# changhaonan/A3VLM

Hardware: AMD Instinct MI355X
Metric: image-text samples/sec (train) + articulation-decode tok/s (higher is better)
Workload: dtype bf16

## Files before the change

a3vlm_amd/csrc/a3v_train.hip:

```cpp
#include "a3v_common.h"

namespace {

template <typename T>
__global__ __launch_bounds__(256) void transpose_kernel(const T* __restrict__ src, int64_t lds_, int64_t bs_s,
                                                        T* __restrict__ dst, int64_t ldd, int64_t bs_d, int R, int C, int Rpad) {
  __shared__ T tile[64][64 + 2];
  const T* s = src + blockIdx.z * bs_s;
  T* d = dst + blockIdx.z * bs_d;
  const int r0 = blockIdx.y * 64, c0 = blockIdx.x * 64;
  const int tx = threadIdx.x & 63, ty = threadIdx.x >> 6;
  for (int i = ty; i < 64; i += 4) {
    const int r = r0 + i, c = c0 + tx;
    tile[i][tx] = (r < R && c < C) ? s[(int64_t)r * lds_ + c] : (T)0.f;
  }
  __syncthreads();
  for (int i = ty; i < 64; i += 4) {
    const int c = c0 + i, r = r0 + tx;
    if (c < C && r < Rpad) d[(int64_t)c * ldd + r] = tile[tx][i];
  }
}

__global__ __launch_bounds__(256) void transpose_bf16_vec_kernel(const bf16_t* __restrict__ src, int64_t lds_, int64_t bs_s,
                                                                 bf16_t* __restrict__ dst, int64_t ldd, int64_t bs_d, int R, int C, int Rpad,
// ... 75 lines not shown
        Cvt<TS>::st(dhr + c, Cvt<TS>::ld(dhr + c) + (r * dyv * w[c] - xv * k2));
        dwp[i] += dyv * xv * r;
      }
    }
  }
  if (dw) {
#pragma unroll
    for (int i = 0; i < MAXC; ++i) {
      const int c = tid + i * 256;
      if (c < dim) atomicAdd(dw + c, dwp[i]);
    }
  }
}


template <typename TA, int RPB, int MAXV, bool PART, typename TS = float>
__global__ __launch_bounds__(256) void rmsnorm_bwd_vec_kernel(const TS* __restrict__ x, int64_t ldx, const float* __restrict__ w,
                                                              const TA* __restrict__ dy, int64_t lddy, TS* __restrict__ dh,
                                                              int64_t lddh, float* __restrict__ dw, int rows, int dim, float eps,
                                                              bf16_t* __restrict__ dh_bf = nullptr, int64_t ld_bf = 0) {
  __shared__ float red[2][8];
  const int tid = threadIdx.x;
  const int nv = dim >> 2;
  f32x4 wv[MAXV], dwp[MAXV];
#pragma unroll
  for (int i = 0; i < MAXV; ++i) {
    const int c = tid + i * 256;
    wv[i] = c < nv ? reinterpret_cast<const f32x4*>(w)[c] : f32x4{0.f, 0.f, 0.f, 0.f};
    dwp[i] = f32x4{0.f, 0.f, 0.f, 0.f};
  }
  const int row0 = blockIdx.x * RPB;
#ifdef RMSB_NO_PREFETCH
  constexpr bool PF = false;
#else
  constexpr bool PF = sizeof(TS) == 2 && sizeof(TA) == 2 && MAXV > 4;
#endif
  bf16x4 nx[MAXV], ng[MAXV], nh[MAXV];
  auto fetch = [&](int row) {
    if constexpr (PF) {
      const int rc = row < rows ? row : rows - 1;
#pragma unroll
      for (int i = 0; i < MAXV; ++i) {
        const int c = tid + i * 256;
        const int cc = c < nv ? c : 0;
        nx[i] = *reinterpret_cast<const bf16x4*>(reinterpret_cast<const bf16_t*>(x) + (int64_t)rc * ldx + 4 * cc);
        ng[i] = *reinterpret_cast<const bf16x4*>(reinterpret_cast<const bf16_t*>(dy) + (int64_t)rc * lddy + 4 * cc);
        nh[i] = *reinterpret_cast<const bf16x4*>(reinterpret_cast<const bf16_t*>(dh) + (int64_t)rc * lddh + 4 * cc);
      }
    }
  };
  fetch(row0);
  for (int rr = 0; rr < RPB; ++rr) {
    const int row = row0 + rr;
    if (row >= rows) break;
    const TS* xr = x + (int64_t)row * ldx;
    const TA* dyr = dy + (int64_t)row * lddy;
    f32x4 xv[MAXV], gv[MAXV], hv[MAXV];
    float s1 = 0.f, s2 = 0.f;
#pragma unroll
    for (int i = 0; i < MAXV; ++i) {
      const int c = tid + i * 256;
      if (c < nv) {
        if constexpr (PF) {
#pragma unroll
          for (int e = 0; e < 4; ++e) { xv[i][e] = (float)nx[i][e]; gv[i][e] = (float)ng[i][e]; hv[i][e] = (float)nh[i][e]; }
        } else {
        if constexpr (sizeof(TS) == 2) {
          const bf16x4 xb = *reinterpret_cast<const bf16x4*>(xr + 4 * c);
#pragma unroll
          for (int e = 0; e < 4; ++e) xv[i][e] = (float)xb[e];
        } else {
          xv[i] = *reinterpret_cast<const f32x4*>(xr + 4 * c);
        }
        if constexpr (sizeof(TA) == 2) {
          const bf16x4 d = *reinterpret_cast<const bf16x4*>(dyr + 4 * c);
#pragma unroll
          for (int e = 0; e < 4; ++e) gv[i][e] = (float)d[e];
        } else {
          gv[i] = *reinterpret_cast<const f32x4*>(dyr + 4 * c);
        }
        }
      } else {
        xv[i] = f32x4{0.f, 0.f, 0.f, 0.f};
        gv[i] = f32x4{0.f, 0.f, 0.f, 0.f};
      }
#pragma unroll
      for (int e = 0; e < 4; ++e) {
        s1 = fmaf(xv[i][e], xv[i][e], s1);
        s2 = fmaf(gv[i][e] * wv[i][e], xv[i][e], s2);
      }
    }
    if (rr + 1 < RPB) fetch(row + 1);
    s1 = wave_sum(s1); s2 = wave_sum(s2);
    const int pb = rr & 1;
    if ((tid & 63) == 0) { red[pb][tid >> 6] = s1; red[pb][4 + (tid >> 6)] = s2; }
    __syncthreads();
    s1 = red[pb][0] + red[pb][1] + red[pb][2] + red[pb][3];
    s2 = red[pb][4] + red[pb][5] + red[pb][6] + red[pb][7];
    const float r = rsqrtf(s1 / (float)dim + eps);
    const float k2 = r * r * r * s2 / (float)dim;
    TS* dhr = dh + (int64_t)row * lddh;
#pragma unroll
    for (int i = 0; i < MAXV; ++i) {
      const int c = tid + i * 256;
      if (c < nv) {
        f32x4 o;
        if constexpr (PF) {
          o = hv[i];
        } else if constexpr (sizeof(TS) == 2) {
          const bf16x4 ob0 = *reinterpret_cast<const bf16x4*>(dhr + 4 * c);
#pragma unroll
          for (int e = 0; e < 4; ++e) o[e] = (float)ob0[e];
        } else {
          o = *reinterpret_cast<const f32x4*>(dhr + 4 * c);
        }
#pragma unroll
        for (int e = 0; e < 4; ++e) {
          o[e] += r * gv[i][e] * wv[i][e] - xv[i][e] * k2;
          dwp[i][e] += gv[i][e] * xv[i][e] * r;
        }
        if constexpr (sizeof(TS) == 2) {
          bf16x4 ob1;
// ... 21 lines not shown
        if (c < nv) out[c] = dwp[i];
      }
    } else {
#pragma unroll
      for (int i = 0; i < MAXV; ++i) {
        const int c = tid + i * 256;
        if (c < nv) {
#pragma unroll
          for (int e = 0; e < 4; ++e) atomicAdd(dw + 4 * c + e, dwp[i][e]);
        }
      }
    }
  }
}

__global__ __launch_bounds__(256) void colsum_add_kernel(const float* __restrict__ part, int nrows, int cols, float* __restrict__ out) {
  const int c = blockIdx.x * 256 + threadIdx.x;
  if (c >= cols) return;
  const int per = (nrows + gridDim.y - 1) / gridDim.y;
  const int r0 = blockIdx.y * per, r1 = min(nrows, r0 + per);
  float a0 = 0.f, a1 = 0.f, a2 = 0.f, a3 = 0.f;
  int r = r0;
  for (; r + 4 <= r1; r += 4) {
    a0 += part[(int64_t)r * cols + c];
    a1 += part[(int64_t)(r + 1) * cols + c];
    a2 += part[(int64_t)(r + 2) * cols + c];
    a3 += part[(int64_t)(r + 3) * cols + c];
  }
  for (; r < r1; ++r) a0 += part[(int64_t)r * cols + c];
  if (r1 > r0) atomicAdd(out + c, (a0 + a1) + (a2 + a3));
}

template <typename TA, int RPB, typename TD = float>
__global__ __launch_bounds__(256) void layernorm_bwd_kernel(const TA* __restrict__ x, int64_t ldx, const float* __restrict__ w,
                                                            const TD* __restrict__ dy, int64_t lddy, const int32_t* __restrict__ row_map,
                                                            TA* __restrict__ dx, int64_t lddx, float* __restrict__ dw, float* __restrict__ db,
                                                            int rows, int dim, float eps) {
  __shared__ float red[12];
  const int tid = threadIdx.x;
  constexpr int MAXC = 32;
  float dwp[MAXC], dbp[MAXC];
#pragma unroll
  for (int i = 0; i < MAXC; ++i) { dwp[i] = 0.f; dbp[i] = 0.f; }
  const int row0 = blockIdx.x * RPB;
  for (int rr = 0; rr < RPB; ++rr) {
// ... 415 lines not shown
static int rmsnorm_bwd_impl(const TS* x, int64_t ldx, const float* w, const void* dy, int64_t lddy, TS* dh, int64_t lddh,
                            float* dw, float* dw_scratch, int rows, int dim, float eps, int act_dtype, void* stream, bf16_t* dh_bf,
                            int64_t ld_bf) {
  if (!x || !w || !dy || !dh || rows <= 0) return A3V_ERR_ARG;
  if (dim > 8192) return A3V_ERR_SHAPE;
  constexpr uintptr_t SMASK = sizeof(TS) == 2 ? 7 : 15;
  if (dim % 4 == 0 && ldx % 4 == 0 && lddy % 4 == 0 && lddh % 4 == 0 && (act_dtype == A3V_BF16 || act_dtype == A3V_F32) &&
      ((reinterpret_cast<uintptr_t>(x) | reinterpret_cast<uintptr_t>(dh)) & SMASK) == 0 && (reinterpret_cast<uintptr_t>(w) & 15) == 0 &&
      (reinterpret_cast<uintptr_t>(dy) & (act_dtype == A3V_BF16 ? 7 : 15)) == 0) {
    constexpr int RV = 8;
    const int nb = (rows + RV - 1) / RV;
    dim3 gv(nb);
    const bool part = dw && dw_scratch && (reinterpret_cast<uintptr_t>(dw_scratch) & 15) == 0;
    float* dwo = part ? dw_scratch : dw;
#define A3V_RB(TT, MV, PP) hipLaunchKernelGGL((rmsnorm_bwd_vec_kernel<TT, RV, MV, PP, TS>), gv, dim3(256), 0, ST, x, ldx, w, (const TT*)dy, lddy, dh, lddh, dwo, rows, dim, eps, dh_bf, ld_bf)
    if (dim <= 4096) {
      if (act_dtype == A3V_BF16) { if (part) A3V_RB(bf16_t, 4, true); else A3V_RB(bf16_t, 4, false); }
      else { if (part) A3V_RB(float, 4, true); else A3V_RB(float, 4, false); }
    } else {
      if (act_dtype == A3V_BF16) { if (part) A3V_RB(bf16_t, 8, true); else A3V_RB(bf16_t, 8, false); }
      else { if (part) A3V_RB(float, 8, true); else A3V_RB(float, 8, false); }
    }
#undef A3V_RB
    A3V_LAUNCH_CHECK();
    if (part) {
      hipLaunchKernelGGL(colsum_add_kernel, dim3((dim + 255) / 256, 16), dim3(256), 0, ST, dw_scratch, nb, dim, dw);
      A3V_LAUNCH_CHECK();
    }
    return A3V_OK;
  }
  constexpr int RPB = 16;
  dim3 g((rows + RPB - 1) / RPB);
  if (act_dtype == A3V_BF16) hipLaunchKernelGGL((rmsnorm_bwd_kernel<bf16_t, RPB, TS>), g, dim3(256), 0, ST, x, ldx, w, (const bf16_t*)dy, lddy, dh, lddh, dw, rows, dim, eps);
  else if (act_dtype == A3V_F32) hipLaunchKernelGGL((rmsnorm_bwd_kernel<float, RPB, TS>), g, dim3(256), 0, ST, x, ldx, w, (const float*)dy, lddy, dh, lddh, dw, rows, dim, eps);
  else return A3V_ERR_DTYPE;
  A3V_LAUNCH_CHECK();
  if (dh_bf) {
    if (sizeof(TS) != 4) return A3V_ERR_ARG;
    return a3v_cast(dh, lddh, A3V_F32, dh_bf, ld_bf, A3V_BF16, rows, dim, stream);
  }
  return A3V_OK;
// ... 361 lines not shown
extern "C" int a3v_lora_gb_scatter(const float* gbt, int64_t ld, int r, int n_mods, float* const* dst, const int* row0, const int* nj, void* stream) {
  if (!gbt || !dst || !row0 || !nj || r <= 0 || n_mods <= 0 || n_mods > 4) return A3V_ERR_ARG;
  GbScatter sc{};
  int mx = 0;
  for (int j = 0; j < n_mods; ++j) {
    if (!dst[j] || nj[j] <= 0 || row0[j] < 0) return A3V_ERR_ARG;
    sc.dst[j] = dst[j]; sc.row0[j] = row0[j]; sc.nj[j] = nj[j];
    mx = nj[j] > mx ? nj[j] : mx;
  }
  hipLaunchKernelGGL(lora_gb_scatter_kernel, dim3((mx * r + 255) / 256, n_mods), dim3(256), 0, (hipStream_t)stream, gbt, ld, r, sc);
  A3V_LAUNCH_CHECK();
  return A3V_OK;
}

namespace {
__global__ __launch_bounds__(256) void adamw_multi_kernel(const a3v_adamw_tensor* __restrict__ tab, float decay, float b1, float b2,
                                                          float step_size, float inv_bc2_sqrt, float eps, const float* __restrict__ gscale) {
  const float gs = gscale ? *gscale : 1.f;
  if (!(gs >= 0.f)) return;
  const a3v_adamw_tensor t = tab[blockIdx.y];
  const int64_t n4 = t.n / 4;
  const int64_t stride = (int64_t)gridDim.x * 256;
  const bool vec_img = t.d1 && !t.d2 && t.s1c == 1 && t.s1r == t.cols && (t.cols & 3) == 0;
  for (int64_t i = (int64_t)blockIdx.x * 256 + threadIdx.x; i < n4; i += stride) {
    f32x4 pp = reinterpret_cast<const f32x4*>(t.p)[i];
    f32x4 gg = reinterpret_cast<const f32x4*>(t.g)[i];
#pragma unroll
    for (int e = 0; e < 4; ++e) gg[e] = __fmul_rn(gg[e], gs);
    f32x4 mm = reinterpret_cast<const f32x4*>(t.m)[i];
    f32x4 vv = reinterpret_cast<const f32x4*>(t.v)[i];
// ... 90 lines not shown
```

a3vlm_amd/lib.py:

```python
from __future__ import annotations

import ctypes
import os
from ctypes import c_float, c_int, c_int64, c_void_p

_HERE = os.path.dirname(os.path.abspath(__file__))
LIB_PATH = os.environ.get("A3V_LIB_PATH") or os.path.join(_HERE, "liba3vlm_hip.so")

BF16, F32 = 0, 1
EPI_NONE, EPI_BIAS, EPI_GELU, EPI_QUICKGELU, EPI_RESIDUAL, EPI_SWIGLU, EPI_OUT_F32, EPI_RES_F32 = 0, 1, 2, 4, 8, 16, 32, 64
EPI_SWIGLU_BWD = 128

EPI_TILE_128, EPI_TILE_256, EPI_TILE_256PP = 1 << 16, 1 << 17, 1 << 18
EPI_TILE_192PP = 1 << 23

P, I, L, F = c_void_p, c_int, c_int64, c_float

SIGNATURES = {
    "a3v_version": (I, []),
    "a3v_reload_env": (I, []),
    "a3v_gemm_nt": (I, [P, L, P, L, P, L, I, I, I, P, P, L, I, I, P]),
    "a3v_gemm_qkv_rope": (I, [P, L, P, L, I, P, L, P, P, P, L, P, L, P, I, I, I, I, I, I, I, I, P]),
    "a3v_gemm_nt_fp8": (I, [P, L, P, P, L, P, P, L, I, I, I, P, P, L, I, P]),
    "a3v_gemm_qkv_rope_fp8": (I, [P, L, P, P, L, P, I, P, L, P, P, P, I, I, I, I, I, I, I, I, P]),
    "a3v_quantize_rows_fp8": (I, [P, L, P, F, P, L, P, I, I, I, P]),
    "a3v_gemm_tn_splitk": (I, [P, L, P, L, P, I, I, I, I, P]),
    "a3v_attention_bwd_packed": (I, [P, P, L, L, P, L, L, L, P, L, P, P, P, P, L, P, I, I, I, I, I, I, I, I, P]),
    "a3v_lora_refresh": (I, [P, P, I, I, I, P, L, P, L, P, L, P, L, I, I, P]),
    "a3v_adamw": (I, [P, P, P, P, L, F, F, F, F, F, L, P, P]),
    "a3v_adamw_scaled": (I, [P, P, P, P, L, F, F, F, F, F, L, P, P, P]),
    "a3v_adamw_scaled_t": (I, [P, P, P, P, I, I, F, F, F, F, F, L, P, P, L, P, P]),
    "a3v_gemm_tn_strip": (I, [P, L, P, L, P, I, I, I, I, P]),
    "a3v_lora_gb_scatter": (I, [P, L, I, I, P, P, P, P]),
    "a3v_adamw_multi": (I, [P, I, L, F, F, F, F, F, L, P, P]),
    "a3v_scale_cast": (I, [P, I, P, I, L, F, P]),
    "a3v_sumsq_partials": (I, [P, L, P, P]),
    "a3v_grad_bucket_allreduce": (I, [P, P, L, P, I, P]),
    "a3v_grad_bucket_reduce_scatter": (I, [P, P, L, P, P, P, I, P]),
    "a3v_param_shard_all_gather": (I, [P, P, P, L, P]),
    "a3v_rccl_comm_count": (I, [P]),
    "a3v_rccl_available": (I, []),
    "a3v_gemm_nn": (I, [P, L, P, L, P, L, I, I, I, P, L, I, P]),
    "a3v_gemm_tn": (I, [P, L, P, L, P, L, I, I, I, P, L, I, P]),
    "a3v_gemm_tn_sumsq": (I, [P, L, P, L, P, L, I, I, I, P, L, I, P, L, P]),
    "a3v_gemm_tn_sumsq_slots": (L, [I, I]),
    "a3v_gemm_set_workspace": (I, [P, L]),
    "a3v_gemm_set_workspace_for": (I, [P, P, L]),
    "a3v_gemm_nt_splitk": (I, [P, L, P, L, P, I, I, I, I, P]),
# ... 118 lines not shown
```

a3vlm_amd/ops.py:

```python
from __future__ import annotations

import ctypes
from typing import Optional

import torch

from . import lib as _l
from .lib import BF16, F32, EPI_BIAS, EPI_GELU, EPI_QUICKGELU, EPI_RESIDUAL, EPI_SWIGLU, EPI_OUT_F32, EPI_RES_F32, EPI_SWIGLU_BWD

_DT = {torch.bfloat16: BF16, torch.float32: F32}


def dt(t: torch.Tensor) -> int:
    try:
        return _DT[t.dtype]
    except KeyError:
        raise TypeError(f"a3vlm_amd supports bf16/fp32 tensors, got {t.dtype}")


def _p(t: Optional[torch.Tensor]):
    return None if t is None else t.data_ptr()


def _stream() -> int:
# ... 96 lines not shown
                               _p(residual), residual.stride(0) if residual is not None else 0, ep, _stream())
    _l.check(rc, f"a3v_gemm_nn(M={M},N={N},K={K},epi={ep})")
    return out


def gemm_tn_strip(t, x, out, scratch, S: int, accumulate: bool = False):
    _dev(t, x, out, scratch)
    Kt, R = t.shape
    N = x.shape[1]
    assert x.shape[0] == Kt and t.stride(1) == 1 and x.stride(1) == 1 and t.stride(0) >= 64
    assert scratch.dtype == torch.float32 and scratch.numel() >= S * R * N
    lib = _l.load()
    _l.check(lib.a3v_gemm_tn_strip(_p(t), t.stride(0), _p(x), x.stride(0), _p(scratch), R, N, Kt, S, _stream()), f"a3v_gemm_tn_strip(R={R},N={N},Kt={Kt},S={S})")
    _l.check(lib.a3v_splitk_reduce(_p(scratch), S, R, N, _p(out), out.stride(0), dt(out), 1 if accumulate else 0, _stream()), "a3v_splitk_reduce")
    return out


def gemm_tn_splitk(at, wt, out, scratch, S: int, accumulate: bool = False):
    _dev(at, wt, out, scratch)
    K, M = at.shape
    N = wt.shape[1]
    assert wt.shape[0] == K and at.stride(1) == 1 and wt.stride(1) == 1
    assert scratch.dtype == torch.float32 and scratch.numel() >= S * M * N
    lib = _l.load()
    _l.check(lib.a3v_gemm_tn_splitk(_p(at), at.stride(0), _p(wt), wt.stride(0), _p(scratch), M, N, K, S, _stream()), f"a3v_gemm_tn_splitk(M={M},N={N},K={K},S={S})")
    _l.check(lib.a3v_splitk_reduce(_p(scratch), S, M, N, _p(out), out.stride(0), dt(out), 1 if accumulate else 0, _stream()), "a3v_splitk_reduce")
    return out


def gemm_skinny_split(M: int, N: int, K: int) -> int:
# ... 408 lines not shown


def lora_gb_scatter(gbt, r: int, views, row0s):
    import ctypes
    _dev(gbt, *views)
    n = len(views)
    assert gbt.dtype == torch.float32 and gbt.stride(1) == 1 and all(v.dtype == torch.float32 and v.is_contiguous() and v.shape[1] == r for v in views)
    dst = (ctypes.c_void_p * n)(*[v.data_ptr() for v in views])
    r0 = (ctypes.c_int * n)(*[int(x) for x in row0s])
    nj = (ctypes.c_int * n)(*[int(v.shape[0]) for v in views])
    rc = _l.load().a3v_lora_gb_scatter(_p(gbt), gbt.stride(0), int(r), n, ctypes.cast(dst, ctypes.c_void_p), ctypes.cast(r0, ctypes.c_void_p),
                                       ctypes.cast(nj, ctypes.c_void_p), _stream())
    _l.check(rc, "a3v_lora_gb_scatter")


def lora_refresh(wa, wb, A, At, B, Bt, col0: int, row0: int):
    _dev(wa, wb, A, At, B, Bt)
    assert wa.dtype == torch.float32 and wb.dtype == torch.float32 and wa.is_contiguous() and wb.is_contiguous()
    assert all(t.dtype == torch.bfloat16 and t.stride(1) == 1 for t in (A, At, B, Bt))
    r, in_f = wa.shape
    nj = wb.shape[0]
    assert wb.shape[1] == r and col0 + r <= A.shape[0] and in_f <= A.shape[1] and row0 + nj <= B.shape[0]
    rc = _l.load().a3v_lora_refresh(_p(wa), _p(wb), r, in_f, nj, _p(A), A.stride(0), _p(At), At.stride(0), _p(B), B.stride(0), _p(Bt),
                                    Bt.stride(0), col0, row0, _stream())
    _l.check(rc, "a3v_lora_refresh")
```

a3vlm_amd/train.py:

```python
from __future__ import annotations

import os

from typing import Callable, Dict, List, Optional, Tuple

import torch

from . import ops
from .util import install_param_epoch_hook, optimizer_steps, param_state_key


def _pad64(n: int) -> int:
    return (n + 63) // 64 * 64


def skinny_slices(M: int, N: int, K: int, cus: int) -> int:
    blocks = ((M + 127) // 128) * ((N + 127) // 128)
    nk = K // 64
    S = 1
    while blocks * S < 512 and S * 2 <= nk and S < 32:
        S *= 2
    if N <= 64 and M >= 2048 and cus > 0 and os.environ.get("A3V_SKINNY_LEGACY", "0") != "1":
        S = max(1, min(cus // ((M + 255) // 256), nk // 2, 32))
    elif N <= 64 and M >= 512 and S > 4:
# ... 20 lines not shown
        if stream_dtype is None:
            stream_dtype = torch.float32 if os.environ.get("A3V_STREAM_FP32", "0") == "1" else compute_dtype
        self.stream = stream_dtype
        self.recompute = recompute
        self._img = None
        self._ws: Dict[tuple, torch.Tensor] = {}
        self._flat: Optional[torch.Tensor] = None
        self._views: Dict[str, torch.Tensor] = {}
        self._ranges: List[Tuple[str, int, int]] = []
        self._fresh: set = set()
        self._gemm_written: set = set()
        self.on_layer_grads_ready: Optional[Callable[[str, int, int], None]] = None
        self.sumsq_sink = None
        self.static_grad_scale: Optional[float] = None
        self._saved = None
        self._weights_ready: Dict[str, torch.cuda.Event] = {}
        self.zero1_world = int(zero1_world or 0)
        if "A3V_NN_DGRAD" not in os.environ:
            self.nn_dgrad = bool(self.zero1_world)
        self._flat_params: Optional[torch.Tensor] = None
        self._z1: List[tuple] = []
        self._z1_fresh = True

    def _buf(self, name, shape, dtype=None, zero=False):
        dtype = dtype or self.act
        key = (name, tuple(shape), dtype)
        t = self._ws.get(key)
        if t is None:
            t = torch.empty(*shape, dtype=dtype, device=self.m._device)
            self._ws[key] = t
# ... 238 lines not shown
        return self._img

    def _wgrad(self, dy: torch.Tensor, x: torch.Tensor, grad: torch.Tensor, tag: str, names=(), store: bool = False):
        M, N = dy.shape
        K = x.shape[1]
        fresh = store or (bool(names) and all(n in self._fresh for n in names))
        assert fresh or not any(n in self._fresh for n in names), "partially fresh fused gradient view"
        tn_ok = (self.tn_wgrad and self.act == torch.bfloat16 and N % 8 == 0 and K % 4 == 0 and dy.stride(0) % 8 == 0
                 and x.stride(0) % 8 == 0 and 2 * M * max(dy.stride(0), x.stride(0)) < 2 ** 31)
        if tn_ok and min(N, K) >= 256:
            self._fresh.difference_update(names if fresh else ())
            sink = self.sumsq_sink
            sq = sink.wgrad_slots(grad, N, K) if sink is not None and grad.is_contiguous() else None
            ops.gemm_tn(dy, x, grad, residual=None if fresh else grad, epilogue=ops.EPI_OUT_F32 if fresh else ops.EPI_RES_F32, sumsq=sq)
            return
        if (tn_ok and self.strip_wgrad and N <= 64 and N % 4 == 0 and K >= 256 and dy.stride(0) >= 64
                and (dy.data_ptr() | x.data_ptr()) % 16 == 0):
            tiles = (K + 127) // 128
            S = max(1, min(64, (M + 63) // 64, -(-512 // tiles)))
            self._fresh.difference_update(names if fresh else ())
            ops.gemm_tn_strip(dy, x, grad, self._buf("splitk", (S * N * K,), torch.float32), S, accumulate=not fresh)
            return
        if tn_ok and min(N, K) <= 64 and max(N, K) >= 256:
            blocks = ((N + 255) // 256) * ((K + 255) // 256)
            S = 1
            while blocks * S < 256 and S < 16 and 2 * S <= (M + 63) // 64:
                S *= 2
            self._fresh.difference_update(names if fresh else ())
            ops.gemm_tn_splitk(dy, x, grad, self._buf("splitk", (S * N * K,), torch.float32), S, accumulate=not fresh)
            return
        Mp = _pad64(M)
        dyt = self._buf("wg_dyt" + tag, (N, Mp))
        xt = self._buf("wg_xt" + tag, (K, Mp))
        ops.transpose(dy, dyt, M, N, Mp)
        ops.transpose(x, xt, M, K, Mp)
        if fresh:
            self._fresh.difference_update(names)
            if min(N, K) <= 64:
                self._skinny(dyt, xt, grad)
            else:
                ops.gemm_nt(dyt, xt, grad, epilogue=ops.EPI_OUT_F32 if self.act == torch.bfloat16 else 0)
        else:
            if min(N, K) <= 64:
                self._skinny(dyt, xt, grad, accumulate=True)
            else:
                ops.gemm_nt(dyt, xt, grad, residual=grad, epilogue=ops.EPI_RES_F32 if self.act == torch.bfloat16 else 0)

    def _skinny(self, a: torch.Tensor, w: torch.Tensor, out: torch.Tensor, accumulate: bool = False):
        M, K = a.shape
        N = w.shape[0]
        S = skinny_slices(M, N, K, self._cus(a.device) if a.is_cuda else 0)
        if S == 1 or self.act != torch.bfloat16 or K % 64:
            f32 = out.dtype == torch.float32 and self.act == torch.bfloat16
            ops.gemm_nt(a, w, out, residual=out if accumulate else None,
                        epilogue=(ops.EPI_RES_F32 if accumulate else ops.EPI_OUT_F32) if f32 else 0)
            return
        ops.gemm_nt_splitk(a, w, out, self._buf("splitk", (S * M * N,), torch.float32), S, accumulate)

    def _cus(self, dev) -> int:
        n = getattr(self, "_cu_count", None)
        if n is None:
# ... 146 lines not shown
        m = self.m
        li = self._lora_step_images()
        r = m.lora_rank
        Bt, At = li[key + ".Bt"], li[key + ".At"]
        M, N = dy.shape
        Rp = t.shape[1]
        if dt is None:
            dt = self._buf("lora_dt", (M, Rp))
            self._dgrad(dy, Bt, dt)
        g = key.split(".")[0]
        names = {"qkv": ["attention.wq", "attention.wk", "attention.wv"], "wo": ["attention.wo"],
                 "w13": ["feed_forward.w1", "feed_forward.w3"], "w2": ["feed_forward.w2"]}[g]
        vas = [self._views[f"layers.{i}.{nm}.lora_a.weight"] for nm in names]
        vbs = [self._views[f"layers.{i}.{nm}.lora_b.weight"] for nm in names]
        nr = len(names) * r
        gBt = self._buf("lora_gBt." + g, (Rp, N), torch.float32)
        self._wgrad(t, dy, gBt, "lb", store=True)
        adjacent = all(vas[j + 1].data_ptr() == vas[j].data_ptr() + 4 * vas[j].numel() for j in range(len(vas) - 1))
        if adjacent and dt.stride(0) % 8 == 0:
            off = (vas[0].data_ptr() - self._flat.data_ptr()) // 4
            self._wgrad(dt[:, :nr], x, self._flat[off:off + nr * x.shape[1]].view(nr, x.shape[1]), "la", store=False)
        else:
            gA = self._buf("lora_gA." + g, (Rp, x.shape[1]), torch.float32)
            self._wgrad(dt, x, gA, "la", store=True)
            for j, va in enumerate(vas):
                ops.add2d(va, gA[j * r:(j + 1) * r])
        row0s, row = [], 0
        for vb in vbs:
            row0s.append(row)
            row += vb.shape[0]
        if gBt.is_cuda:
            ops.lora_gb_scatter(gBt, r, vbs, row0s)
        else:
# ... 197 lines not shown
            ops.attention_bwd(k["qrot"], k["kc"], Hkv * spad * hd, spad * hd, vrows, S * ld, ld, hd, att_c, datt, k["lse"], D,
                              dq, dk, dv, B, S, H, Hkv, hd, True, workspace=wsp)
            ops.rope_bwd_pack(dq, dk, dv, dqkv, m._cos_sin_dev(), B, S, H, Hkv, hd, 0)
        if self._has(pre + "attention.wq.weight", pre + "attention.wk.weight", pre + "attention.wv.weight"):
            self._wgrad(dqkv, k["xn"], self._gview(pre + "attention.wq.weight", pre + "attention.wv.weight"), "qkv",
                        (pre + "attention.wq.weight", pre + "attention.wk.weight", pre + "attention.wv.weight"))
        if kx:
            self._kx_group_bwd(i, f"qkv.{i}", dqkv_full, (H + 2 * Hkv) * hd, k["xn"], lt["qkv"], dxn)
        else:
            self._dgrad_w(dqkv, f"qkv.{i}", dxn)
            if self.lora:
                self._lora_bwd(i, f"qkv.{i}", dqkv, k["xn"], lt["qkv"], dxn)
        ops.rmsnorm_bwd(h_in, l.attention_norm.weight, dxn, dh, self._views.get(pre + "attention_norm.weight"), a.norm_eps,
                        dh_lowp=dha if fuse_cast else None)
        self._dha_ready = fuse_cast

    @torch.no_grad()
    def forward_loss(self, examples: torch.Tensor, labels: torch.Tensor, image: Optional[torch.Tensor] = None,
                     qformer_feats=None, extra_feats=None) -> torch.Tensor:
        self._check_dtypes()
        self._li_checked = False
        m, a = self.m, self.m.args
        im = self._images()
        B, T = examples.shape
        n_img = 0 if image is None else (len(image) if isinstance(image, (list, tuple)) else 1)
        W = m.words_per_image * n_img if n_img else 0
        S = T + W
        rows = B * S
        dim, V = a.dim, a.vocab_size
        h = self._buf("h", (rows, dim), self.stream)
# ... 37 lines not shown
        n_valid = self._buf("n_valid", (1,), torch.int32)
        ops.count_valid(lab, n_valid)
        row_loss = self._buf("row_loss", (B * T,), torch.float32)
        ops.cross_entropy(logits, lab, row_loss)
        nv = n_valid.to(torch.float32)[0]
        loss = torch.where(nv > 0, row_loss.sum() / torch.clamp(nv, min=1.0), torch.zeros_like(nv))
        self._saved = dict(B=B, T=T, W=W, S=S, h=h, hs=hs, xt=xt, logits=logits, lab=lab, n_valid=n_valid, tokens=examples.contiguous(), vis=vis,
                           kept=kept if not self.recompute else None)
        return loss

    @torch.no_grad()
    def backward(self, grad_scale: float = 1.0) -> None:
        s = self._saved
        self._dha_ready = False
        self._li_checked = False
        assert s is not None, "backward() without forward_loss()"
        m, a = self.m, self.m.args
        self.sync_optimizer()
        im = self._images()
        self.ensure_grads()
        if not self.nn_dgrad and not self.lora and not getattr(self, "_nt_mem_checked", False):
            self._nt_mem_checked = True
            need = 2 * sum(q.numel() for g_ in im.groups() if g_ != "vp" for q in im._params(g_)[0])
            if not getattr(self, "_opt_stepped", False):
                need += 8 * sum(q.numel() for q in m.parameters() if q.requires_grad)
            free, _ = torch.cuda.mem_get_info(m._device)
            free += torch.cuda.memory_reserved(m._device) - torch.cuda.memory_allocated(m._device)
            if free - need < 8 * 2 ** 30 or (self.recompute and "A3V_NN_DGRAD" not in os.environ):
                self.nn_dgrad = True
        if self.lora and not getattr(self, "_nt_mem_checked", False):
# ... 326 lines not shown
```

include/a3vlm_hip.h:

```cpp
#ifndef A3VLM_HIP_H
#define A3VLM_HIP_H

#include <stdint.h>

#ifdef __cplusplus
extern "C" {
#endif

enum { A3V_BF16 = 0, A3V_F32 = 1 };

enum {
  A3V_OK = 0,
  A3V_ERR_SHAPE = -1,
  A3V_ERR_DTYPE = -2,
  A3V_ERR_ARG = -3
};

enum {
  A3V_EPI_NONE = 0,
  A3V_EPI_BIAS = 1,
  A3V_EPI_GELU = 2,
  A3V_EPI_QUICKGELU = 4,
  A3V_EPI_RESIDUAL = 8,
  A3V_EPI_SWIGLU = 16,
// ... 205 lines not shown
                  int W, int dim, int vocab, void* stream);

int a3v_rows_sum(const void* src, int64_t ld, const int32_t* row_idx, int n_rows, int dim, float* out,
                 int dtype, void* stream);

int a3v_adamw(float* param, const float* grad, float* exp_avg, float* exp_avg_sq, int64_t n, float lr, float beta1, float beta2,
              float eps, float weight_decay, int64_t step, void* bf16_image, void* stream);

int a3v_adamw_scaled(float* param, const float* grad, float* exp_avg, float* exp_avg_sq, int64_t n, float lr, float beta1, float beta2,
                     float eps, float weight_decay, int64_t step, void* bf16_image, const float* grad_scale, void* stream);

int a3v_lora_gb_scatter(const float* gbt, int64_t ld, int r, int n_mods, float* const* dst, const int* row0, const int* nj, void* stream);

int a3v_gemm_tn_strip(const void* T, int64_t ldt, const void* X, int64_t ldx, float* partial, int R, int N, int Kt, int S, void* stream);

int a3v_adamw_scaled_t(float* param, const float* grad, float* exp_avg, float* exp_avg_sq, int rows, int cols, float lr, float beta1,
                       float beta2, float eps, float weight_decay, int64_t step, void* bf16_image, void* bf16_image_t, int64_t ldt,
                       const float* grad_scale, void* stream);

typedef struct {
  float* p; const float* g; float* m; float* v;
  int64_t n, cols;
  void* d1; int64_t s1r, s1c;
  void* d2; int64_t s2r, s2c;
} a3v_adamw_tensor;
int a3v_adamw_multi(const a3v_adamw_tensor* table, int n_tensors, int64_t max_n, float lr, float beta1, float beta2, float eps,
                    float weight_decay, int64_t step, const float* grad_scale, void* stream);

int a3v_scale_cast(const void* src, int src_dtype, void* dst, int dst_dtype, int64_t n, float scale, void* stream);

// ... 19 lines not shown
```

Baseline: 35.96.

## Batch LoRA gradient split-K reductions into one per-layer finish kernel

LoRA A/B weight gradients are computed as strip split-K partial planes, and their reduction, transpose and scatter into the parameter views are deferred into a single job-table kernel launched once per layer after the attention norm backward. This removes the separate per-projection splitk-reduce and scatter launches. The rmsnorm backward gains a form selector that issues the dh load early for small dims. The dw column-sum now reduces chunks in shared memory instead of using atomics. The job table is cached per layer keyed by pointers, so the host builds it once and reuses it.

```diff
diff --git a/a3vlm_amd/csrc/a3v_train.hip b/a3vlm_amd/csrc/a3v_train.hip
--- a/a3vlm_amd/csrc/a3v_train.hip
+++ b/a3vlm_amd/csrc/a3v_train.hip
@@ -113,7 +113,7 @@
 }
 
 
-template <typename TA, int RPB, int MAXV, bool PART, typename TS = float>
+template <typename TA, int RPB, int MAXV, bool PART, typename TS = float, int FORM = -1>
 __global__ __launch_bounds__(256) void rmsnorm_bwd_vec_kernel(const TS* __restrict__ x, int64_t ldx, const float* __restrict__ w,
                                                               const TA* __restrict__ dy, int64_t lddy, TS* __restrict__ dh,
                                                               int64_t lddh, float* __restrict__ dw, int rows, int dim, float eps,
@@ -132,8 +132,9 @@
 #ifdef RMSB_NO_PREFETCH
   constexpr bool PF = false;
 #else
-  constexpr bool PF = sizeof(TS) == 2 && sizeof(TA) == 2 && MAXV > 4;
+  constexpr bool PF = sizeof(TS) == 2 && sizeof(TA) == 2 && (FORM < 0 ? MAXV > 4 : FORM == 2);
 #endif
+  constexpr bool EARLY = !PF && FORM == 1;
   bf16x4 nx[MAXV], ng[MAXV], nh[MAXV];
   auto fetch = [&](int row) {
     if constexpr (PF) {
@@ -155,6 +156,7 @@
     const TS* xr = x + (int64_t)row * ldx;
     const TA* dyr = dy + (int64_t)row * lddy;
     f32x4 xv[MAXV], gv[MAXV], hv[MAXV];
+    bf16x4 hraw[MAXV];
     float s1 = 0.f, s2 = 0.f;
 #pragma unroll
     for (int i = 0; i < MAXV; ++i) {
@@ -177,6 +179,14 @@
           for (int e = 0; e < 4; ++e) gv[i][e] = (float)d[e];
         } else {
           gv[i] = *reinterpret_cast<const f32x4*>(dyr + 4 * c);
+        }
+        if constexpr (EARLY) {
+          const TS* hr = dh + (int64_t)row * lddh;
+          if constexpr (sizeof(TS) == 2) {
+            hraw[i] = *reinterpret_cast<const bf16x4*>(hr + 4 * c);
+          } else {
+            hv[i] = *reinterpret_cast<const f32x4*>(hr + 4 * c);
+          }
         }
         }
       } else {
@@ -204,7 +214,10 @@
       const int c = tid + i * 256;
       if (c < nv) {
         f32x4 o;
-        if constexpr (PF) {
+        if constexpr (EARLY && sizeof(TS) == 2) {
+#pragma unroll
+          for (int e = 0; e < 4; ++e) o[e] = (float)hraw[i][e];
+        } else if constexpr (PF || EARLY) {
           o = hv[i];
         } else if constexpr (sizeof(TS) == 2) {
           const bf16x4 ob0 = *reinterpret_cast<const bf16x4*>(dhr + 4 * c);
@@ -256,21 +269,33 @@
   }
 }
 
-__global__ __launch_bounds__(256) void colsum_add_kernel(const float* __restrict__ part, int nrows, int cols, float* __restrict__ out) {
-  const int c = blockIdx.x * 256 + threadIdx.x;
-  if (c >= cols) return;
-  const int per = (nrows + gridDim.y - 1) / gridDim.y;
-  const int r0 = blockIdx.y * per, r1 = min(nrows, r0 + per);
+constexpr int CSA_COLS = 32, CSA_CHUNKS = 16;
+__global__ __launch_bounds__(CSA_COLS * CSA_CHUNKS) void colsum_add_kernel(const float* __restrict__ part, int nrows, int cols,
+                                                                           float* __restrict__ out) {
+  __shared__ float sums[CSA_CHUNKS][CSA_COLS];
+  const int lc = threadIdx.x & (CSA_COLS - 1), chunk = threadIdx.x / CSA_COLS;
+  const int c = blockIdx.x * CSA_COLS + lc;
+  const int per = (nrows + CSA_CHUNKS - 1) / CSA_CHUNKS;
+  const int r0 = min(nrows, chunk * per), r1 = min(nrows, r0 + per);
   float a0 = 0.f, a1 = 0.f, a2 = 0.f, a3 = 0.f;
-  int r = r0;
-  for (; r + 4 <= r1; r += 4) {
-    a0 += part[(int64_t)r * cols + c];
-    a1 += part[(int64_t)(r + 1) * cols + c];
-    a2 += part[(int64_t)(r + 2) * cols + c];
-    a3 += part[(int64_t)(r + 3) * cols + c];
-  }
-  for (; r < r1; ++r) a0 += part[(int64_t)r * cols + c];
-  if (r1 > r0) atomicAdd(out + c, (a0 + a1) + (a2 + a3));
+  if (c < cols) {
+    int r = r0;
+    for (; r + 4 <= r1; r += 4) {
+      a0 += part[(int64_t)r * cols + c];
+      a1 += part[(int64_t)(r + 1) * cols + c];
+      a2 += part[(int64_t)(r + 2) * cols + c];
+      a3 += part[(int64_t)(r + 3) * cols + c];
+    }
+    for (; r < r1; ++r) a0 += part[(int64_t)r * cols + c];
+  }
+  sums[chunk][lc] = (a0 + a1) + (a2 + a3);
+  __syncthreads();
+  if (chunk == 0 && c < cols) {
+    float o = out[c];
+    for (int k = 0; k < CSA_CHUNKS; ++k)
+      if (min(nrows, k * per) < min(nrows, k * per + per)) o += sums[k][lc];
+    out[c] = o;
+  }
 }
 
 template <typename TA, int RPB, typename TD = float>
@@ -716,6 +741,17 @@
     const bool part = dw && dw_scratch && (reinterpret_cast<uintptr_t>(dw_scratch) & 15) == 0;
     float* dwo = part ? dw_scratch : dw;
 #define A3V_RB(TT, MV, PP) hipLaunchKernelGGL((rmsnorm_bwd_vec_kernel<TT, RV, MV, PP, TS>), gv, dim3(256), 0, ST, x, ldx, w, (const TT*)dy, lddy, dh, lddh, dwo, rows, dim, eps, dh_bf, ld_bf)
+    const int form_env = A3V_ENV_INT("A3V_RMSB_FORM", -1);
+    const int form = form_env >= 0 && form_env <= 2 ? form_env : (dim <= 4096 ? 1 : 2);
+    if constexpr (sizeof(TS) == 2) {
+      if (act_dtype != A3V_BF16) return A3V_ERR_DTYPE;
+#define A3V_RBF(MV, PP, FM) hipLaunchKernelGGL((rmsnorm_bwd_vec_kernel<bf16_t, RV, MV, PP, TS, FM>), gv, dim3(256), 0, ST, x, ldx, w, (const bf16_t*)dy, lddy, dh, lddh, dwo, rows, dim, eps, dh_bf, ld_bf)
+#define A3V_RBF3(MV, PP) do { if (form == 0) A3V_RBF(MV, PP, 0); else if (form == 1) A3V_RBF(MV, PP, 1); else A3V_RBF(MV, PP, 2); } while (0)
+      if (dim <= 4096) { if (part) A3V_RBF3(4, true); else A3V_RBF3(4, false); }
+      else { if (part) A3V_RBF3(8, true); else A3V_RBF3(8, false); }
+#undef A3V_RBF3
+#undef A3V_RBF
+    } else
     if (dim <= 4096) {
       if (act_dtype == A3V_BF16) { if (part) A3V_RB(bf16_t, 4, true); else A3V_RB(bf16_t, 4, false); }
       else { if (part) A3V_RB(float, 4, true); else A3V_RB(float, 4, false); }
@@ -726,7 +762,7 @@
 #undef A3V_RB
     A3V_LAUNCH_CHECK();
     if (part) {
-      hipLaunchKernelGGL(colsum_add_kernel, dim3((dim + 255) / 256, 16), dim3(256), 0, ST, dw_scratch, nb, dim, dw);
+      hipLaunchKernelGGL(colsum_add_kernel, dim3((dim + CSA_COLS - 1) / CSA_COLS), dim3(CSA_COLS * CSA_CHUNKS), 0, ST, dw_scratch, nb, dim, dw);
       A3V_LAUNCH_CHECK();
     }
     return A3V_OK;
@@ -1118,6 +1154,116 @@
 }
 
 namespace {
+constexpr int LGF_ROWS = 16, LGF_COLS = 128, LGF_LD = LGF_COLS + 4;
+constexpr int LGF_MAX_JOBS = 64;
+
+__host__ __device__ inline int64_t lgf_dst_tiles(const a3v_lora_grad_dst& d) {
+  return ((d.r1 - d.r0 + LGF_ROWS - 1) / LGF_ROWS) * ((d.n + LGF_COLS - 1) / LGF_COLS);
+}
+
+__global__ __launch_bounds__(256) void lora_grad_finish_kernel(const a3v_lora_grad_job* __restrict__ jobs, int n_jobs) {
+  __shared__ __attribute__((aligned(16))) float patch[LGF_ROWS * LGF_LD];
+  const int tid = threadIdx.x;
+  int ji = 0;
+  while (ji + 1 < n_jobs && (int64_t)blockIdx.x >= jobs[ji + 1].block0) ++ji;
+  const a3v_lora_grad_job* jb = jobs + ji;
+  int rem = (int)((int64_t)blockIdx.x - jb->block0);
+  int di = 0;
+  const int nd = (int)jb->n_dst;
+  for (; di < nd; ++di) {
+    const int t = (int)lgf_dst_tiles(jb->dst[di]);
+    if (rem < t) break;
+    rem -= t;
+  }
+  if (di >= nd) return;
+  const a3v_lora_grad_dst d = jb->dst[di];
+  const int S = (int)jb->S, R = (int)jb->R, N = (int)jb->N;
+  const int r = (int)(d.r1 - d.r0), ncol = (int)d.n;
+  const int ctiles = (ncol + LGF_COLS - 1) / LGF_COLS;
+  const int rt = rem / ctiles, ct = rem - rt * ctiles;
+  const int lc = ct * LGF_COLS + (tid & 31) * 4;
+  const int lr0 = rt * LGF_ROWS + (tid >> 5);
+  const bool cok = lc < ncol;
+  const bool ok0 = cok && lr0 < r, ok1 = cok && lr0 + 8 < r;
+  const int64_t plane = (int64_t)R * N;
+  const float* p0 = jb->planes + (int64_t)(d.r0 + lr0) * N + d.c0 + lc;
+  const float* p1 = p0 + (int64_t)8 * N;
+  f32x4 a0 = {0.f, 0.f, 0.f, 0.f}, a1 = {0.f, 0.f, 0.f, 0.f};
+  for (int s0 = 0; s0 < S; s0 += 8) {
+    f32x4 x0[8], x1[8];
+#pragma unroll
+    for (int u = 0; u < 8; ++u) {
+      const bool in = s0 + u < S;
+      x0[u] = ok0 && in ? *reinterpret_cast<const f32x4*>(p0 + (int64_t)(s0 + u) * plane) : f32x4{0.f, 0.f, 0.f, 0.f};
+      x1[u] = ok1 && in ? *reinterpret_cast<const f32x4*>(p1 + (int64_t)(s0 + u) * plane) : f32x4{0.f, 0.f, 0.f, 0.f};
+    }
+#pragma unroll
+    for (int u = 0; u < 8; ++u) {
+      if (s0 + u < S) {
+#pragma unroll
+        for (int e = 0; e < 4; ++e) { a0[e] += x0[u][e]; a1[e] += x1[u][e]; }
+      }
+    }
+  }
+#pragma unroll
+  for (int e = 0; e < 4; ++e) { a0[e] = rbf(a0[e]); a1[e] = rbf(a1[e]); }
+  if (d.kind == 0) {
+    if (ok0) {
+      f32x4* o = reinterpret_cast<f32x4*>(d.dst + (int64_t)lr0 * d.ld + lc);
+      if (d.accumulate) { const f32x4 h = *o; *o = h + a0; } else *o = a0;
+    }
+    if (ok1) {
+      f32x4* o = reinterpret_cast<f32x4*>(d.dst + (int64_t)(lr0 + 8) * d.ld + lc);
+      if (d.accumulate) { const f32x4 h = *o; *o = h + a1; } else *o = a1;
+    }
+    return;
+  }
+  const int prow = tid >> 5, pcol = (tid & 31) * 4;
+  *reinterpret_cast<f32x4*>(patch + prow * LGF_LD + pcol) = a0;
+  *reinterpret_cast<f32x4*>(patch + (prow + 8) * LGF_LD + pcol) = a1;
+  __syncthreads();
+#pragma unroll
+  for (int pass = 0; pass < 2; ++pass) {
+    const int idx = tid + 256 * pass;
+    const int nn = idx >> 2, q = idx & 3;
+    const int col = ct * LGF_COLS + nn, row = rt * LGF_ROWS + 4 * q;
+    if (col < ncol && row < r) {
+      f32x4 v;
+#pragma unroll
+      for (int e = 0; e < 4; ++e) v[e] = patch[(4 * q + e) * LGF_LD + nn];
+      f32x4* o = reinterpret_cast<f32x4*>(d.dst + (int64_t)col * r + row);
+      if (d.accumulate) { const f32x4 h = *o; *o = h + v; } else *o = v;
+    }
+  }
+}
+}
+
+extern "C" int a3v_lora_grad_finish(const a3v_lora_grad_job* jobs_host, const a3v_lora_grad_job* jobs_dev, int n_jobs, void* stream) {
+  if (!jobs_host || !jobs_dev || n_jobs <= 0 || n_jobs > LGF_MAX_JOBS) return A3V_ERR_ARG;
+  if (reinterpret_cast<uintptr_t>(jobs_dev) & 7) return A3V_ERR_ARG;
+  int64_t blocks = 0;
+  for (int j = 0; j < n_jobs; ++j) {
+    const a3v_lora_grad_job& jb = jobs_host[j];
+    if (!jb.planes || jb.S < 1 || jb.S > 64 || jb.R <= 0 || jb.N <= 0 || jb.n_dst < 1 || jb.n_dst > 3) return A3V_ERR_ARG;
+    if (jb.block0 != blocks) return A3V_ERR_ARG;
+    if ((jb.N & 3) || (reinterpret_cast<uintptr_t>(jb.planes) & 15)) return A3V_ERR_SHAPE;
+    if (jb.S * jb.R * jb.N * 4 >= (1LL << 31)) return A3V_ERR_SHAPE;
+    for (int k = 0; k < jb.n_dst; ++k) {
+      const a3v_lora_grad_dst& d = jb.dst[k];
+      if (!d.dst || (d.kind != 0 && d.kind != 1) || d.r0 < 0 || d.r1 <= d.r0 || d.r1 > jb.R || d.c0 < 0 || d.n <= 0 || d.c0 + d.n > jb.N) return A3V_ERR_ARG;
+      if (((d.r1 - d.r0) & 3) || (d.c0 & 3) || (d.n & 3) || (reinterpret_cast<uintptr_t>(d.dst) & 15)) return A3V_ERR_SHAPE;
+      if (d.kind == 0 && (d.ld < d.n || (d.ld & 3) || (d.r1 - d.r0) * d.ld * 4 >= (1LL << 31))) return A3V_ERR_SHAPE;
+      if (d.kind == 1 && d.n * (d.r1 - d.r0) * 4 >= (1LL << 31)) return A3V_ERR_SHAPE;
+      blocks += lgf_dst_tiles(d);
+    }
+  }
+  if (blocks <= 0 || blocks >= (1LL << 31)) return A3V_ERR_SHAPE;
+  hipLaunchKernelGGL(lora_grad_finish_kernel, dim3((unsigned)blocks), dim3(256), 0, (hipStream_t)stream, jobs_dev, n_jobs);
+  A3V_LAUNCH_CHECK();
+  return A3V_OK;
+}
+
+namespace {
 __global__ __launch_bounds__(256) void adamw_multi_kernel(const a3v_adamw_tensor* __restrict__ tab, float decay, float b1, float b2,
                                                           float step_size, float inv_bc2_sqrt, float eps, const float* __restrict__ gscale) {
   const float gs = gscale ? *gscale : 1.f;
diff --git a/a3vlm_amd/lib.py b/a3vlm_amd/lib.py
--- a/a3vlm_amd/lib.py
+++ b/a3vlm_amd/lib.py
@@ -32,6 +32,7 @@
     "a3v_adamw_scaled_t": (I, [P, P, P, P, I, I, F, F, F, F, F, L, P, P, L, P, P]),
     "a3v_gemm_tn_strip": (I, [P, L, P, L, P, I, I, I, I, P]),
     "a3v_lora_gb_scatter": (I, [P, L, I, I, P, P, P, P]),
+    "a3v_lora_grad_finish": (I, [P, P, I, P]),
     "a3v_adamw_multi": (I, [P, I, L, F, F, F, F, F, L, P, P]),
     "a3v_scale_cast": (I, [P, I, P, I, L, F, P]),
     "a3v_sumsq_partials": (I, [P, L, P, P]),
diff --git a/a3vlm_amd/ops.py b/a3vlm_amd/ops.py
--- a/a3vlm_amd/ops.py
+++ b/a3vlm_amd/ops.py
@@ -134,6 +134,16 @@
     _l.check(lib.a3v_gemm_tn_strip(_p(t), t.stride(0), _p(x), x.stride(0), _p(scratch), R, N, Kt, S, _stream()), f"a3v_gemm_tn_strip(R={R},N={N},Kt={Kt},S={S})")
     _l.check(lib.a3v_splitk_reduce(_p(scratch), S, R, N, _p(out), out.stride(0), dt(out), 1 if accumulate else 0, _stream()), "a3v_splitk_reduce")
     return out
+
+
+def gemm_tn_strip_planes(t, x, planes, S: int):
+    _dev(t, x, planes)
+    Kt, R = t.shape
+    N = x.shape[1]
+    assert x.shape[0] == Kt and t.stride(1) == 1 and x.stride(1) == 1 and t.stride(0) >= 64
+    assert planes.dtype == torch.float32 and planes.is_contiguous() and planes.numel() >= S * R * N
+    _l.check(_l.load().a3v_gemm_tn_strip(_p(t), t.stride(0), _p(x), x.stride(0), _p(planes), R, N, Kt, S, _stream()),
+             f"a3v_gemm_tn_strip(R={R},N={N},Kt={Kt},S={S})")
 
 
 def gemm_tn_splitk(at, wt, out, scratch, S: int, accumulate: bool = False):
@@ -572,6 +582,40 @@
     _l.check(rc, "a3v_lora_gb_scatter")
 
 
+LGF_PLAIN, LGF_TRANSPOSED = 0, 1
+_LGF_ROWS, _LGF_COLS = 16, 128
+
+
+class LoraGradTable:
+
+    def __init__(self, jobs, key=None):
+        import numpy as np
+        rows, block0, keep = [], 0, []
+        for planes, S, R, N, dsts in jobs:
+            assert planes.dtype == torch.float32 and planes.is_contiguous() and planes.numel() >= S * R * N and 1 <= len(dsts) <= 3
+            row = [planes.data_ptr(), int(S), int(R), int(N), block0, len(dsts)]
+            keep.append(planes)
+            for kind, dst, ld, acc, r0, r1, c0, n in dsts:
+                assert dst.dtype == torch.float32 and dst.stride(-1) == 1
+                row += [dst.data_ptr(), int(ld), int(kind), 1 if acc else 0, int(r0), int(r1), int(c0), int(n)]
+                block0 += -(-(r1 - r0) // _LGF_ROWS) * -(-n // _LGF_COLS)
+                keep.append(dst)
+            row += [0] * (8 * (3 - len(dsts)))
+            rows.append(row)
+        _dev(*keep)
+        self.n = len(rows)
+        self.host = np.ascontiguousarray(np.array(rows, dtype=np.int64))
+        self.dev = torch.from_numpy(self.host).to(keep[0].device)
+        self.blocks = block0
+        self.key = key
+        self._keep = keep
+
+
+def lora_grad_finish(table: LoraGradTable):
+    rc = _l.load().a3v_lora_grad_finish(table.host.ctypes.data, table.dev.data_ptr(), table.n, _stream())
+    _l.check(rc, f"a3v_lora_grad_finish(jobs={table.n},blocks={table.blocks})")
+
+
 def lora_refresh(wa, wb, A, At, B, Bt, col0: int, row0: int):
     _dev(wa, wb, A, At, B, Bt)
     assert wa.dtype == torch.float32 and wb.dtype == torch.float32 and wa.is_contiguous() and wb.is_contiguous()
diff --git a/a3vlm_amd/train.py b/a3vlm_amd/train.py
--- a/a3vlm_amd/train.py
+++ b/a3vlm_amd/train.py
@@ -58,6 +58,9 @@
         self.sumsq_sink = None
         self.static_grad_scale: Optional[float] = None
         self._saved = None
+        self.lora_grad_batch = os.environ.get("A3V_LORA_GRAD_BATCH", "1") != "0"
+        self._lgf_jobs: list = []
+        self._lgf_tables: Dict[int, "ops.LoraGradTable"] = {}
         self._weights_ready: Dict[str, torch.cuda.Event] = {}
         self.zero1_world = int(zero1_world or 0)
         if "A3V_NN_DGRAD" not in os.environ:
@@ -326,10 +329,8 @@
             sq = sink.wgrad_slots(grad, N, K) if sink is not None and grad.is_contiguous() else None
             ops.gemm_tn(dy, x, grad, residual=None if fresh else grad, epilogue=ops.EPI_OUT_F32 if fresh else ops.EPI_RES_F32, sumsq=sq)
             return
-        if (tn_ok and self.strip_wgrad and N <= 64 and N % 4 == 0 and K >= 256 and dy.stride(0) >= 64
-                and (dy.data_ptr() | x.data_ptr()) % 16 == 0):
-            tiles = (K + 127) // 128
-            S = max(1, min(64, (M + 63) // 64, -(-512 // tiles)))
+        S = self._strip_slices(dy, x) if tn_ok else 0
+        if S:
             self._fresh.difference_update(names if fresh else ())
             ops.gemm_tn_strip(dy, x, grad, self._buf("splitk", (S * N * K,), torch.float32), S, accumulate=not fresh)
             return
@@ -357,6 +358,53 @@
                 self._skinny(dyt, xt, grad, accumulate=True)
             else:
                 ops.gemm_nt(dyt, xt, grad, residual=grad, epilogue=ops.EPI_RES_F32 if self.act == torch.bfloat16 else 0)
+
+    def _strip_slices(self, dy: torch.Tensor, x: torch.Tensor) -> int:
+        M, N = dy.shape
+        K = x.shape[1]
+        if not (self.strip_wgrad and N <= 64 and N % 4 == 0 and K >= 256 and dy.stride(0) >= 64 and (dy.data_ptr() | x.data_ptr()) % 16 == 0):
+            return 0
+        tiles = (K + 127) // 128
+        return max(1, min(64, (M + 63) // 64, -(-512 // tiles)))
+
+    def _lora_strips_batched(self, i: int, g: str, t, dy, dt, x, vas, vbs, r: int) -> bool:
+        nr = len(vas) * r
+        M = dy.shape[0]
+        if not (self.lora_grad_batch and self.tn_wgrad and self.act == torch.bfloat16 and dy.is_cuda and r % 4 == 0 and nr % 8 == 0
+                and nr <= t.shape[1]):
+            return False
+        tb, ta = t[:, :nr], dt[:, :nr]
+        for u, v in ((tb, dy), (ta, x)):
+            if not (v.shape[1] % 4 == 0 and u.stride(0) % 8 == 0 and v.stride(0) % 8 == 0 and 2 * M * max(u.stride(0), v.stride(0)) < 2 ** 31):
+                return False
+        Sb, Sa = self._strip_slices(tb, dy), self._strip_slices(ta, x)
+        if not Sb or not Sa or any(vb.shape[0] % 4 or not vb.is_contiguous() or vb.data_ptr() % 16 for vb in vbs) or vas[0].data_ptr() % 16:
+            return False
+        N, K = dy.shape[1], x.shape[1]
+        pb = self._buf("lgf_b." + g, (Sb * nr * N,), torch.float32)
+        pa = self._buf("lgf_a." + g, (Sa * nr * K,), torch.float32)
+        ops.gemm_tn_strip_planes(tb, dy, pb, Sb)
+        ops.gemm_tn_strip_planes(ta, x, pa, Sa)
+        off = (vas[0].data_ptr() - self._flat.data_ptr()) // 4
+        ga = self._flat[off:off + nr * K].view(nr, K)
+        dsts, row = [], 0
+        for j, vb in enumerate(vbs):
+            dsts.append((ops.LGF_TRANSPOSED, vb, r, True, j * r, (j + 1) * r, row, vb.shape[0]))
+            row += vb.shape[0]
+        self._lgf_jobs.append((pb, Sb, nr, N, dsts))
+        self._lgf_jobs.append((pa, Sa, nr, K, [(ops.LGF_PLAIN, ga, K, True, 0, nr, 0, K)]))
+        return True
+
+    def _lora_grads_finish(self, i: int) -> None:
+        jobs, self._lgf_jobs = self._lgf_jobs, []
+        if not jobs:
+            return
+        key = tuple((p.data_ptr(), S, R, N, tuple((k, d.data_ptr(), ld, acc, r0, r1, c0, n) for k, d, ld, acc, r0, r1, c0, n in ds))
+                    for p, S, R, N, ds in jobs)
+        tab = self._lgf_tables.get(i)
+        if tab is None or tab.key != key:
+            tab = self._lgf_tables[i] = ops.LoraGradTable(jobs, key)
+        ops.lora_grad_finish(tab)
 
     def _skinny(self, a: torch.Tensor, w: torch.Tensor, out: torch.Tensor, accumulate: bool = False):
         M, K = a.shape
@@ -533,9 +581,13 @@
         vas = [self._views[f"layers.{i}.{nm}.lora_a.weight"] for nm in names]
         vbs = [self._views[f"layers.{i}.{nm}.lora_b.weight"] for nm in names]
         nr = len(names) * r
+        adjacent = all(vas[j + 1].data_ptr() == vas[j].data_ptr() + 4 * vas[j].numel() for j in range(len(vas) - 1))
+        if adjacent and dt.stride(0) % 8 == 0 and self._lora_strips_batched(i, g, t, dy, dt, x, vas, vbs, r):
+            if dx is not None:
+                ops.gemm_nt(dt, At, dx, residual=dx)
+            return
         gBt = self._buf("lora_gBt." + g, (Rp, N), torch.float32)
         self._wgrad(t, dy, gBt, "lb", store=True)
-        adjacent = all(vas[j + 1].data_ptr() == vas[j].data_ptr() + 4 * vas[j].numel() for j in range(len(vas) - 1))
         if adjacent and dt.stride(0) % 8 == 0:
             off = (vas[0].data_ptr() - self._flat.data_ptr()) // 4
             self._wgrad(dt[:, :nr], x, self._flat[off:off + nr * x.shape[1]].view(nr, x.shape[1]), "la", store=False)
@@ -763,6 +815,7 @@
         ops.rmsnorm_bwd(h_in, l.attention_norm.weight, dxn, dh, self._views.get(pre + "attention_norm.weight"), a.norm_eps,
                         dh_lowp=dha if fuse_cast else None)
         self._dha_ready = fuse_cast
+        self._lora_grads_finish(i)
 
     @torch.no_grad()
     def forward_loss(self, examples: torch.Tensor, labels: torch.Tensor, image: Optional[torch.Tensor] = None,
@@ -830,6 +883,7 @@
         s = self._saved
         self._dha_ready = False
         self._li_checked = False
+        self._lgf_jobs = []
         assert s is not None, "backward() without forward_loss()"
         m, a = self.m, self.m.args
         self.sync_optimizer()
diff --git a/include/a3vlm_hip.h b/include/a3vlm_hip.h
--- a/include/a3vlm_hip.h
+++ b/include/a3vlm_hip.h
@@ -243,6 +243,19 @@
 
 int a3v_gemm_tn_strip(const void* T, int64_t ldt, const void* X, int64_t ldx, float* partial, int R, int N, int Kt, int S, void* stream);
 
+typedef struct {
+  float* dst; int64_t ld;
+  int64_t kind, accumulate;
+  int64_t r0, r1, c0, n;
+} a3v_lora_grad_dst;
+typedef struct {
+  const float* planes;
+  int64_t S, R, N;
+  int64_t block0, n_dst;
+  a3v_lora_grad_dst dst[3];
+} a3v_lora_grad_job;
+int a3v_lora_grad_finish(const a3v_lora_grad_job* jobs_host, const a3v_lora_grad_job* jobs_dev, int n_jobs, void* stream);
+
 int a3v_adamw_scaled_t(float* param, const float* grad, float* exp_avg, float* exp_avg_sq, int rows, int cols, float lr, float beta1,
                        float beta2, float eps, float weight_decay, int64_t step, void* bf16_image, void* bf16_image_t, int64_t ldt,
                        const float* grad_scale, void* stream);
```

Measured after the change: 36.22 (median of 6 runs). No clear change (+0.7%).
